# filaPro/unidet3d

Hardware: AMD Instinct MI355X
Metric: scenes/sec fwd+bwd, 100k-pt ScanNet voxel grid, 1/2/4/8 MI355X (higher is better)
Workload: dtype f32

## Files before the change

include/u3d.h:

```cpp
#ifndef U3D_H_
#define U3D_H_

#include <stdint.h>

#ifdef __cplusplus
extern "C" {
#endif

typedef void* u3d_stream_t;

#define U3D_OK 0
#define U3D_EINVAL (-1)
#define U3D_ELAUNCH (-2)
#define U3D_EUNSUPPORTED (-3)

#define U3D_ABI_VERSION 117
int u3d_version(void);
const char* u3d_last_error(void);
int u3d_fp32_math(int mode);

int u3d_conv_kernel(int mode);

int u3d_attn_tile_waves(int waves);

// ... 221 lines not shown
int u3d_attn_varlen_bwd_drop_b16(const void* qkv, const void* out, const void* dout, const float* lse, const int32_t* cu_seqlens,
                                 int B, int max_len, int64_t n_total, int H, int hd, float scale, void* dqkv, float* delta_ws,
                                 double flops_hint, u3d_stream_t stream, double p, uint64_t seed, uint64_t offset);
int u3d_dropout_mask_attn(double p, uint64_t seed, uint64_t offset, int H, int64_t n_total, uint8_t* mask ,
                          u3d_stream_t stream);
int u3d_dropout_mask_rows(double p, uint64_t seed, uint64_t offset, int64_t n, int C, uint8_t* mask , u3d_stream_t stream);
int u3d_dropout_fwd(const float* x, float* y, int64_t n, int C, double p, uint64_t seed, uint64_t offset, u3d_stream_t stream);
int u3d_dropout_bwd(const float* dy, float* dx, int64_t n, int C, double p, uint64_t seed, uint64_t offset, u3d_stream_t stream);
int u3d_dropout_fwd_b16(const void* x, void* y, int64_t n, int C, double p, uint64_t seed, uint64_t offset, u3d_stream_t stream);
int u3d_dropout_bwd_b16(const void* dy, void* dx, int64_t n, int C, double p, uint64_t seed, uint64_t offset, u3d_stream_t stream);

int u3d_gemm_nt(const float* A , const float* W , const float* bias , float* C ,
                int64_t M, int N, int K , const void* w_planes, double flops_hint, u3d_stream_t stream);
#define U3D_BF16_OPERANDS 16
int u3d_linear_act(const float* X , const float* W , const float* bias, int act, float* pre, float* Y ,
                   int64_t M, int N, int K, const void* w_planes, double flops_hint, u3d_stream_t stream);
int u3d_linear_dact(const float* dY , const float* Wt , const float* aux, int act, float* dX ,
                    int64_t M, int N, int K, const void* w_planes, double flops_hint, u3d_stream_t stream);
int u3d_gemm_nt_add(const float* A , const float* W , const float* addend , int flags, float* C, int64_t M,
                    int N, int K, const void* w_planes, double flops_hint, u3d_stream_t stream);
int u3d_ln_linear(const float* X, const float* RES, const float* gamma, const float* beta, float eps, float* SUM, float* NQ, float* STATS,
                  const float* W , const float* bias, int act, float* PRE, float* Y , int64_t M, int C, int N,
                  const void* w_planes, double flops_hint, u3d_stream_t stream);
int u3d_ffn_fwd(const float* X, const float* W1 , const float* b1, const float* W2 , const float* b2,
                int act, float* H, float* A, float* Z , int64_t M, int d_in, int hid, int d_out,
                const void* w1_planes, const void* w2_planes, double flops_hint, u3d_stream_t stream);
int u3d_gelu_fwd(const float* h, float* a, int64_t n, u3d_stream_t stream);
int u3d_gelu_bwd(const float* da, const float* h, float* dh, int64_t n, u3d_stream_t stream);
int u3d_gemm_tn(const float* A , const float* B , float* C , float* colsum_A, int64_t M, int N, int K,
                void* ws, double flops_hint, u3d_stream_t stream);
int u3d_gemm_tn_bf16(const float* A, const float* B, float* C, float* colsum_A, int64_t M, int N, int K, void* ws, double flops_hint,
                     u3d_stream_t stream);
int64_t u3d_gemm_tn_ws_bytes(int64_t M, int N, int K);
int u3d_transpose(const float* in , float* out , int R, int C, u3d_stream_t stream);
int u3d_transpose_batch(const void* desc, int n_desc, int64_t total_blocks, u3d_stream_t stream);
int u3d_weight_planes_batch(const void* desc, int n_desc, int64_t total_blocks, u3d_stream_t stream);

#define U3D_A_BF16 1
#define U3D_B_BF16 2
#define U3D_C_BF16 4
int u3d_gemm_nt_b16(const void* A, const float* W, const float* bias, int epi, const void* aux, void* C, int flags, int64_t M, int N, int K,
                    double flops_hint, u3d_stream_t stream);
int u3d_gemm_tn_b16(const void* A, const void* B, float* C, float* colsum_A, int flags, int64_t M, int N, int K, void* ws, double flops_hint,
                    u3d_stream_t stream);
int64_t u3d_gemm_tn_b16_ws_bytes(int64_t M, int N, int K);
int u3d_gelu_fwd_b16(const void* h, void* a, int64_t n, u3d_stream_t stream);
int u3d_gelu_bwd_b16(const void* da, const void* h, void* dh, int64_t n, u3d_stream_t stream);

#define U3D_GEMM_NATIVE 0
#define U3D_GEMM_X3 1
#define U3D_GEMM_B16 2
int u3d_gemm_nt_plan(int64_t M, int N, int K, int flags, int* kernel, int* tile_m, int* tile_n);
int u3d_gemm_nt_b16_plan(int64_t M, int N, int K, int epi, int flags, int* tile_m, int* tile_n);
int u3d_gemm_tn_plan(int64_t M, int N, int K, int bf16_operands, int* kernel, int* tile_n, int* tile_k, int* splits, int64_t* rows_per_split);
int u3d_gemm_tn_b16_plan(int64_t M, int N, int K, int flags, int* tile_n, int* tile_k, int* splits, int64_t* rows_per_split);

int u3d_layer_norm_fwd(const float* x, const float* res, const float* gamma, const float* beta, int64_t M, int C, float eps,
                       float* sum_out, float* y, float* stats, u3d_stream_t stream);
int u3d_layer_norm_bwd(const float* s, const float* dy, const float* gamma, const float* stats, int64_t M, int C, float* dx,
                       float* dgamma, float* dbeta, void* ws, u3d_stream_t stream);
int u3d_layer_norm_fwd_b16(const float* x, const float* res, const float* gamma, const float* beta, int64_t M, int C, float eps,
                           float* sum_out, float* y, void* y16, float* stats, u3d_stream_t stream);
int u3d_layer_norm_bwd_b16(const float* s, const float* dy, const float* gamma, const float* stats, int64_t M, int C, float* dx, void* dx16,
                           float* dgamma, float* dbeta, void* ws, u3d_stream_t stream);
int u3d_layer_norm_bwd_sum(const float* s, const float* dy, const float* dy2, const float* dy3, const float* gamma, const float* stats,
                           int64_t M, int C, float* dx, void* dx16, float* dgamma, float* dbeta, void* ws, u3d_stream_t stream);
// ... 96 lines not shown
```

unidet3d_amd/_lib.py:

```python
from __future__ import annotations

import ctypes as C
import os

import torch

_HERE = os.path.dirname(os.path.abspath(__file__))
LIB_PATH = os.environ.get('U3D_LIB_PATH') or os.path.join(_HERE, 'csrc', 'libu3d_hip.so')

_vp, _i32, _i64, _f32, _f64 = C.c_void_p, C.c_int, C.c_int64, C.c_float, C.c_double
_u64 = C.c_uint64


class ConvEpilogue(C.Structure):
    _fields_ = [('raw', _vp), ('raw_ld', _i64), ('raw_col', _i64), ('n_act', _i32), ('act', _vp * 2), ('scale', _vp * 2), ('shift', _vp * 2),
                ('act_ld', _i64 * 2), ('act_col', _i64 * 2), ('relu', _i32 * 2)]


PROTOTYPES = {
    'u3d_version': (_i32, []),
    'u3d_last_error': (C.c_char_p, []),
    'u3d_fp32_math': (_i32, [_i32]),
    'u3d_conv_kernel': (_i32, [_i32]),
    'u3d_attn_tile_waves': (_i32, [_i32]),
    'u3d_prof_enable': (_i32, [_i32, _i32]),
    'u3d_prof_collect': (_i32, [_i32, C.POINTER(_f64), C.POINTER(_i64), C.POINTER(_f64)]),
    'u3d_vox_scene_stats': (_i32, [_vp, _vp, _vp, _i32, _i64, _f32, _i32, _vp, _vp, _vp, _vp]),
    'u3d_vox_scene_stats_ws_bytes': (_i64, [_i32]),
    'u3d_index_words': (_i64, [_i32, _i32, _i32, _i32]),
    'u3d_vox_mark': (_i32, [_vp, _vp, _vp, _i32, _i64, _vp, _f32, _i32, _i32, _i32, _i32, _vp, _vp, _vp]),
    'u3d_index_rank': (_i32, [_vp, _i64, _vp, _vp, _vp]),
    'u3d_index_rank_ws_bytes': (_i64, [_i64]),
    'u3d_index_coords': (_i32, [_vp, _vp, _i32, _i32, _i32, _i32, _vp, _vp]),
    'u3d_vox_finalize': (_i32, [_vp, _vp, _i32, _i64, _vp, _vp, _vp, _vp, _i64, _i64, _vp, _vp, _vp, _vp, _i32, _vp, _vp]),
    'u3d_hash_index_slots': (_i64, [_i64]),
    'u3d_hash_index_ws_bytes': (_i64, [_i64]),
    'u3d_hash_index_build': (_i32, [_vp, _i64, _i64, _vp, _vp, _vp, _vp, _i64, _vp, _vp]),
    'u3d_sort_u64': (_i32, [_vp, _i64, _i32, _vp, _vp, _vp, _vp]),
    'u3d_sort_ws_bytes': (_i64, [_i64, _i32]),
    'u3d_hash_index_coords': (_i32, [_vp, _i64, _i32, _i32, _i32, _vp, _vp]),
    'u3d_cells_of_coords': (_i32, [_vp, _i64, _i32, _i32, _i32, _i32, _i32, _vp, _vp]),
    'u3d_vox_finalize_ws_bytes': (_i64, [_i64, _i64]),
    'u3d_subm_rulebook': (_i32, [_vp, _i64, _vp, _vp, _i64, _i32, _i32, _i32, _i32, _vp, _vp, _vp, _vp, _vp]),
    'u3d_subm_rulebook_ws_bytes': (_i64, [_i64]),
    'u3d_index_mark': (_i32, [_vp, _i64, _i32, _i32, _i32, _i32, _vp, _vp]),
    'u3d_down_rulebook': (_i32, [_vp, _i64, _vp, _vp, _i64, _i32, _i32, _i32, _i32, _vp, _vp, _vp, _vp, _vp]),
    'u3d_down_rulebook_ws_bytes': (_i64, [_i64]),
    'u3d_conv_out_shape': (_i32, [C.POINTER(_i32), _i32, _i32, _i32, C.POINTER(_i32)]),
    'u3d_conv_mark': (_i32, [_vp, _i64, C.POINTER(_i32), _i32, _i32, _i32, _i32, _vp, _vp, _vp]),
# ... 68 lines not shown
    'u3d_relu_bwd': (_i32, [_vp, _vp, _i64, _vp, _vp]),
    'u3d_rows_take': (_i32, [_vp, _vp, _i64, _i64, _i32, _vp, _vp]),
    'u3d_rows_take2': (_i32, [_vp, _vp, _i64, _vp, _vp, _i64, _i64, _i32, _vp, _vp]),
    'u3d_segment_gather_sum': (_i32, [_vp, _vp, _vp, _i64, _i32, _i32, _vp, _vp, _vp]),
    'u3d_segment_mean_xyz': (_i32, [_vp, _i32, _vp, _vp, _i64, _vp, _i32, _vp, _i32, _vp, _vp]),
    'u3d_segment_minmax_xyz': (_i32, [_vp, _i32, _vp, _i64, _i32, _vp, _i32, _vp, _i32, _vp, _vp, _vp]),
    'u3d_criterion_packed': (_i32, [_vp] * 11 + [_i32, _i32, _i64, _i32, _i32, _i64, _i64, _i32, _i32, _f32, _f32, _f32, _f32, _f32, _vp, _vp, _vp, _vp, _vp]),
    'u3d_box_decode_fwd': (_i32, [_vp, _vp, _i64, _vp, _vp]),
    'u3d_box_decode_bwd': (_i32, [_vp, _vp, _i64, _vp, _vp]),
    'u3d_box_decode7_fwd': (_i32, [_vp, _vp, _vp, _i64, _vp, _vp]),
    'u3d_box_decode7_bwd': (_i32, [_vp, _vp, _vp, _i64, _vp, _vp]),
    'u3d_criterion_ws_bytes': (_i64, [_i32, _i32, _i64, _i64, _i64]),
    'u3d_criterion_ws_bytes_gt': (_i64, [_i32, _i32, _i64, _i64, _i64, _i32]),
    'u3d_gemm_nt': (_i32, [_vp, _vp, _vp, _vp, _i64, _i32, _i32, _vp, _f64, _vp]),
    'u3d_linear_act': (_i32, [_vp, _vp, _vp, _i32, _vp, _vp, _i64, _i32, _i32, _vp, _f64, _vp]),
    'u3d_linear_dact': (_i32, [_vp, _vp, _vp, _i32, _vp, _i64, _i32, _i32, _vp, _f64, _vp]),
    'u3d_gemm_nt_add': (_i32, [_vp, _vp, _vp, _i32, _vp, _i64, _i32, _i32, _vp, _f64, _vp]),
    'u3d_ln_linear': (_i32, [_vp, _vp, _vp, _vp, _f32, _vp, _vp, _vp, _vp, _vp, _i32, _vp, _vp, _i64, _i32, _i32, _vp, _f64, _vp]),
    'u3d_ffn_fwd': (_i32, [_vp, _vp, _vp, _vp, _vp, _i32, _vp, _vp, _vp, _i64, _i32, _i32, _i32, _vp, _vp, _f64, _vp]),
    'u3d_gelu_fwd': (_i32, [_vp, _vp, _i64, _vp]),
    'u3d_gelu_bwd': (_i32, [_vp, _vp, _vp, _i64, _vp]),
    'u3d_gemm_nt_b16': (_i32, [_vp, _vp, _vp, _i32, _vp, _vp, _i32, _i64, _i32, _i32, _f64, _vp]),
    'u3d_gemm_tn_b16': (_i32, [_vp, _vp, _vp, _vp, _i32, _i64, _i32, _i32, _vp, _f64, _vp]),
    'u3d_gemm_tn_b16_ws_bytes': (_i64, [_i64, _i32, _i32]),
    'u3d_gelu_fwd_b16': (_i32, [_vp, _vp, _i64, _vp]),
    'u3d_gelu_bwd_b16': (_i32, [_vp, _vp, _vp, _i64, _vp]),
    'u3d_gemm_nt_plan': (_i32, [_i64, _i32, _i32, _i32, C.POINTER(_i32), C.POINTER(_i32), C.POINTER(_i32)]),
    'u3d_gemm_nt_b16_plan': (_i32, [_i64, _i32, _i32, _i32, _i32, C.POINTER(_i32), C.POINTER(_i32)]),
    'u3d_gemm_tn_plan': (_i32, [_i64, _i32, _i32, _i32, C.POINTER(_i32), C.POINTER(_i32), C.POINTER(_i32), C.POINTER(_i32), C.POINTER(_i64)]),
    'u3d_gemm_tn_b16_plan': (_i32, [_i64, _i32, _i32, _i32, C.POINTER(_i32), C.POINTER(_i32), C.POINTER(_i32), C.POINTER(_i64)]),
    'u3d_gemm_tn': (_i32, [_vp, _vp, _vp, _vp, _i64, _i32, _i32, _vp, _f64, _vp]),
    'u3d_gemm_tn_bf16': (_i32, [_vp, _vp, _vp, _vp, _i64, _i32, _i32, _vp, _f64, _vp]),
    'u3d_gemm_tn_ws_bytes': (_i64, [_i64, _i32, _i32]),
    'u3d_transpose': (_i32, [_vp, _vp, _i32, _i32, _vp]),
    'u3d_transpose_batch': (_i32, [_vp, _i32, _i64, _vp]),
    'u3d_weight_planes_batch': (_i32, [_vp, _i32, _i64, _vp]),
    'u3d_attn_varlen_fwd': (_i32, [_vp, _vp, _i32, _i32, _i64, _i32, _i32, _f32, _vp, _vp, _f64, _vp]),
    'u3d_attn_varlen_bwd': (_i32, [_vp, _vp, _vp, _vp, _vp, _i32, _i32, _i64, _i32, _i32, _f32, _vp, _vp, _f64, _vp]),
    'u3d_attn_varlen_fwd_bf16': (_i32, [_vp, _vp, _i32, _i32, _i64, _i32, _i32, _f32, _vp, _vp, _f64, _vp]),
    'u3d_attn_varlen_bwd_bf16': (_i32, [_vp, _vp, _vp, _vp, _vp, _i32, _i32, _i64, _i32, _i32, _f32, _vp, _vp, _f64, _vp]),
    'u3d_attn_varlen_fwd_b16': (_i32, [_vp, _vp, _i32, _i32, _i64, _i32, _i32, _f32, _vp, _vp, _f64, _vp]),
    'u3d_attn_varlen_bwd_b16': (_i32, [_vp, _vp, _vp, _vp, _vp, _i32, _i32, _i64, _i32, _i32, _f32, _vp, _vp, _f64, _vp]),
    'u3d_attn_varlen_fwd_drop': (_i32, [_vp, _vp, _i32, _i32, _i64, _i32, _i32, _f32, _vp, _vp, _f64, _vp, _f64, _u64, _u64]),
    'u3d_attn_varlen_bwd_drop': (_i32, [_vp, _vp, _vp, _vp, _vp, _i32, _i32, _i64, _i32, _i32, _f32, _vp, _vp, _f64, _vp, _f64, _u64, _u64]),
    'u3d_attn_varlen_fwd_drop_bf16': (_i32, [_vp, _vp, _i32, _i32, _i64, _i32, _i32, _f32, _vp, _vp, _f64, _vp, _f64, _u64, _u64]),
    'u3d_attn_varlen_bwd_drop_bf16': (_i32, [_vp, _vp, _vp, _vp, _vp, _i32, _i32, _i64, _i32, _i32, _f32, _vp, _vp, _f64, _vp, _f64, _u64, _u64]),
    'u3d_attn_varlen_fwd_drop_b16': (_i32, [_vp, _vp, _i32, _i32, _i64, _i32, _i32, _f32, _vp, _vp, _f64, _vp, _f64, _u64, _u64]),
    'u3d_attn_varlen_bwd_drop_b16': (_i32, [_vp, _vp, _vp, _vp, _vp, _i32, _i32, _i64, _i32, _i32, _f32, _vp, _vp, _f64, _vp, _f64, _u64, _u64]),
    'u3d_dropout_mask_attn': (_i32, [_f64, _u64, _u64, _i32, _i64, _vp, _vp]),
    'u3d_dropout_mask_rows': (_i32, [_f64, _u64, _u64, _i64, _i32, _vp, _vp]),
    'u3d_dropout_fwd': (_i32, [_vp, _vp, _i64, _i32, _f64, _u64, _u64, _vp]),
    'u3d_dropout_bwd': (_i32, [_vp, _vp, _i64, _i32, _f64, _u64, _u64, _vp]),
    'u3d_dropout_fwd_b16': (_i32, [_vp, _vp, _i64, _i32, _f64, _u64, _u64, _vp]),
    'u3d_dropout_bwd_b16': (_i32, [_vp, _vp, _i64, _i32, _f64, _u64, _u64, _vp]),
    'u3d_aug_points': (_i32, [_vp, _i64, _vp, _vp, _vp, _i32, _i64, _vp, C.POINTER(_f32), C.POINTER(_f32), _f32, _vp, _vp, _vp]),
    'u3d_aug_extent_f32': (_i32, [_vp, _vp, _i32, _i64, _vp, _vp]),
    'u3d_aug_extent_f64': (_i32, [_vp, _vp, _i32, _i64, _vp, _vp]),
    'u3d_aug_noise_blur': (_i32, [_vp, _vp, _vp, _i32, _i64, _vp, _vp, _vp]),
    'u3d_aug_noise_blur_ws_bytes': (_i64, [_i64]),
    'u3d_aug_elastic': (_i32, [_vp, _i32, _vp, _i32, _vp, _i32, _i64, _vp, _vp, _vp, _vp, _f64, _f64, _vp]),
    'u3d_relabel_ids': (_i32, [_vp, _i64, _vp, _vp, _vp, _i32, _i64, _vp, _i64, _i32, _vp, _vp, _i32, _vp, _vp, _vp, _vp, _vp, _vp]),
    'u3d_relabel_ids_ws_bytes': (_i64, [_i64]),
    'u3d_aug_remap_ids': (_i32, [_vp, _vp, _i32, _i64, _vp, _vp, _vp]),
    'u3d_aug_sp_masks': (_i32, [_vp, _vp, _vp, _i64, _vp, _i32, _i64, _vp, _vp, _vp, _i64, _i64, _vp, _vp, _vp]),
    'u3d_aug_sp_masks_ws_bytes': (_i64, [_i64, _i64]),
    'u3d_aug_points_dn': (_i32, [_vp, _i64, _vp, _vp, _vp, _i32, _i64, _vp, C.POINTER(_f32), C.POINTER(_f32), C.POINTER(_f32), C.POINTER(_f32),
# ... 80 lines not shown
    if torch.device(device).type != 'cuda':
        return t.to(device)
    return t.pin_memory().to(device, non_blocking=True)


def h2d_pack(specs, device):
    parts, off = [], 0
    for values, dtype in specs:
        t = torch.tensor(values, dtype=dtype).reshape(-1)
        parts.append((t, off))
        off = (off + t.numel() * t.element_size() + 15) // 16 * 16
    host = torch.empty(max(off, 16), dtype=torch.uint8)
    if torch.device(device).type == 'cuda':
        host = host.pin_memory()
    for t, o in parts:
        if t.numel():
            host[o:o + t.numel() * t.element_size()].view(t.dtype).copy_(t)
    dev = host.to(device, non_blocking=True)
    return [dev[o:o + t.numel() * t.element_size()].view(t.dtype) for t, o in parts]


_SCRATCH = {}


def scratch(nbytes: int, device) -> torch.Tensor:
    key = (device, stream())
    t = _SCRATCH.get(key)
    if t is None or t.numel() < nbytes:
        t = torch.empty(max(int(nbytes), 1 << 21), dtype=torch.uint8, device=device)
        _SCRATCH[key] = t
    return t


def prof_enable(cls: int, on: bool):
    call('u3d_prof_enable', cls, 1 if on else 0)


def prof_collect(cls: int):
    ms, n, w = _f64(), _i64(), _f64()
    call('u3d_prof_collect', cls, C.byref(ms), C.byref(n), C.byref(w))
    return ms.value, n.value, w.value
```

unidet3d_amd/csrc/gemm.hip:

```cpp
#include "gemm_common.h"

namespace u3d {

#define U3D_MFMA32(a, b, c) __builtin_amdgcn_mfma_f32_32x32x2f32((a), (b), (c), 0, 0, 0)

constexpr int GLD = GK + 4;


template <int TN, int EPI, int TM = GT>
__global__ __launch_bounds__(256) void gemm_nt_k(const float* __restrict__ A, const float* __restrict__ W, const float* __restrict__ bias,
                                                 float* __restrict__ C, int64_t M, int N, int K, const float* __restrict__ aux,
                                                 float* __restrict__ pre) {
    constexpr int NB = TN / 64, TA = TM / 64;
    __shared__ __attribute__((aligned(16))) float As[2][TM * GLD];
    __shared__ __attribute__((aligned(16))) float Bs[2][TN * GLD];
    const int tid = threadIdx.x, lane = tid & 63;
    const int wave = __builtin_amdgcn_readfirstlane(tid >> 6);
    const int wr = wave >> 1, wc = wave & 1, i32 = lane & 31, kh = lane >> 5;
    const int nt_ = (N + TN - 1) / TN;
    const int64_t wid_ = xcd_swizzle(blockIdx.x, gridDim.x);
    const int64_t m0 = (wid_ / nt_) * TM;
    const int n0 = (int)(wid_ % nt_) * TN;
    const int rows_a = (int)min((int64_t)TM, M - m0), rows_b = min(TN, N - n0);
    const __amdgpu_buffer_rsrc_t rs_a = make_rsrc(A + m0 * K, (int64_t)rows_a * K * 4);
// ... 419 lines not shown
            lstore();
            if (t + 2 < nt) gload(t + 2);
        }
        __syncthreads();
    }
    const int64_t pstride = (int64_t)N * K + (colsum ? N : 0);
    const __amdgpu_buffer_rsrc_t rs_o = make_rsrc(partial + (int64_t)split * pstride, (int64_t)N * K * 4);
#pragma unroll
    for (int b = 0; b < NB; ++b) {
        const int k = k0 + 16 * (wc * NB + b) + t16;
        const int vo = k < K ? ((n0 + 4 * g) * K + k) * 4 : 0x7fffffff;
#pragma unroll
        for (int a = 0; a < NA; ++a)
#pragma unroll
            for (int r = 0; r < 4; ++r) {
                float v = acc[a][b][r] + lo[a][b][r];
                asm volatile("" : "+v"(v));
                __builtin_amdgcn_raw_buffer_store_b32(__builtin_bit_cast(unsigned, v), rs_o, vo, (16 * (wr * NA + a) + r) * K * 4, 0);
            }
    }
    if (colsum && k0 == 0) {
#pragma unroll
        for (int c = 0; c < 4; ++c) csum_s[rowa][ca4 * 4 + c] = cs[c];
        __syncthreads();
        if (tid < TA && n0 + tid < N) {
            float v = 0.f;
#pragma unroll
            for (int r = 0; r < RPA; ++r) v += csum_s[r][tid];
            partial[(int64_t)split * pstride + (int64_t)N * K + n0 + tid] = v;
        }
    }
}


__global__ __launch_bounds__(256) void gemm_tn_bf16_k(const float* __restrict__ A, const float* __restrict__ B, float* __restrict__ partial,
                                                      int colsum, int64_t M, int N, int K, int64_t rows_per_split) {
    __shared__ __attribute__((aligned(16))) __bf16 As[2][TKH * TLH];
    __shared__ __attribute__((aligned(16))) __bf16 Bs[2][TKH * TLH];
    __shared__ float csum_s[8][GT];
    const int tid = threadIdx.x, lane = tid & 63;
    const int wave = __builtin_amdgcn_readfirstlane(tid >> 6);
    const int wr = wave >> 1, wc = wave & 1, i32 = lane & 31, kh = lane >> 5;
    const int n0 = blockIdx.x * GT, k0 = blockIdx.y * GT;
    const int64_t mlo = (int64_t)blockIdx.z * rows_per_split;
    const int64_t mhi = min(M, mlo + rows_per_split);
    const int rows = (int)max((int64_t)0, mhi - mlo);
    const int srow = tid >> 5, sc4 = tid & 31;
    const __amdgpu_buffer_rsrc_t rs_a = make_rsrc(A + mlo * N, (int64_t)rows * N * 4);
    const __amdgpu_buffer_rsrc_t rs_b = make_rsrc(B + mlo * K, (int64_t)rows * K * 4);
    const int va = n0 + sc4 * 4 < N ? (srow * N + n0 + sc4 * 4) * 4 : 0x7fffffff;
    const int vb = k0 + sc4 * 4 < K ? (srow * K + k0 + sc4 * 4) * 4 : 0x7fffffff;
    const bool ca = va != 0x7fffffff, cb = vb != 0x7fffffff;
    f32x4 ra[4], rb[4];
    f32x4 cs = {0.f, 0.f, 0.f, 0.f};
    auto gload = [&](int t) {
#pragma unroll
        for (int j = 0; j < 4; ++j) {
            ra[j] = bload128(rs_a, ca ? va + j * 8 * N * 4 : va, t * (TKH * N * 4));
            rb[j] = bload128(rs_b, cb ? vb + j * 8 * K * 4 : vb, t * (TKH * K * 4));
        }
    };
    auto lstore = [&](int buf) {
#pragma unroll
        for (int j = 0; j < 4; ++j) {
            cs += ra[j];
            *reinterpret_cast<bf16x4*>(&As[buf][(srow + 8 * j) * TLH + sc4 * 4]) = bf16x4{(__bf16)ra[j][0], (__bf16)ra[j][1], (__bf16)ra[j][2], (__bf16)ra[j][3]};
// ... 219 lines not shown
        case 0: launch_nt<0>(A, W, bias, C, M, N, K, aux, pre, plan, s, wplanes); break;
        case 1: launch_nt<1>(A, W, bias, C, M, N, K, aux, pre, plan, s, wplanes); break;
        case 2: launch_nt<2>(A, W, bias, C, M, N, K, aux, pre, plan, s, wplanes); break;
        case 3: launch_nt<3>(A, W, bias, C, M, N, K, aux, pre, plan, s, wplanes); break;
        case 4: launch_nt<4>(A, W, bias, C, M, N, K, aux, pre, plan, s, wplanes); break;
        default: launch_nt<5>(A, W, bias, C, M, N, K, aux, pre, plan, s, wplanes); break;
    }
    return check_launch("gemm_nt");
}

static bool tn_x3_on() { static const int on = [] { const char* e = getenv("U3D_TN_X3"); return e ? atoi(e) : 1; }(); return on != 0 && fp32_x3(); }
static int tn_x3_ta(int N, int K) { return tn_tile(N, K) == GT ? 128 : 64; }
static int tn_x3_splits(int64_t M, int N, int K) {
    const int64_t tiles = ceil_div(N, tn_x3_ta(N, K)) * ceil_div(K, 64);
    return tn_clamp_splits(ceil_div(768, tiles), M, TXK);
}

static int tn_plan(int64_t M, int N, int K, bool bf, TnPlan* plan) {
    if (M <= 0 || N <= 0 || K <= 0) return U3D_EINVAL;
    if (N % 4 || K % 4) { set_error("gemm_tn: N=%d, K=%d must be multiples of 4", N, K); return U3D_EUNSUPPORTED; }
    const bool x3 = !bf && tn_x3_on();
    const int T = bf ? GT : tn_tile(N, K);
    const int S = x3 ? tn_x3_splits(M, N, K) : tn_splits(M, N, K, T, bf);
    const int64_t rps = x3 ? ceil_div(ceil_div(M, S), TXK) * TXK : ceil_div(ceil_div(M, S), GK) * GK;
    if (!tn_offsets_ok("gemm_tn", M, N, K, rps)) return U3D_EUNSUPPORTED;
    plan->kernel = x3 ? U3D_GEMM_X3 : (bf ? U3D_GEMM_B16 : U3D_GEMM_NATIVE);
    plan->ta = x3 ? tn_x3_ta(N, K) : T;
    plan->tb = x3 ? 64 : T;
    plan->splits = S;
    plan->rows_per_split = rps;
    return U3D_OK;
}

}

using namespace u3d;

extern "C" {


int u3d_gemm_nt(const float* A, const float* W, const float* bias, float* C, int64_t M, int N, int K, const void* w_planes, double flops_hint,
                u3d_stream_t stream) {
    return gemm_nt_epi(A, W, bias, C, M, N, K, 0, nullptr, nullptr, w_planes, flops_hint, (hipStream_t)stream);
}

int u3d_linear_act(const float* X, const float* W, const float* bias, int act, float* pre, float* Y, int64_t M, int N, int K,
                   const void* w_planes, double flops_hint, u3d_stream_t stream) {
    const int bf = (act & U3D_BF16_OPERANDS) ? 8 : 0;
    act &= ~U3D_BF16_OPERANDS;
    if (act < 0 || act > 2) return U3D_EINVAL;
    return gemm_nt_epi(X, W, bias, Y, M, N, K, act | bf, nullptr, pre, w_planes, flops_hint, (hipStream_t)stream);
}

int u3d_linear_dact(const float* dY, const float* Wt, const float* aux, int act, float* dX, int64_t M, int N, int K, const void* w_planes,
                    double flops_hint, u3d_stream_t stream) {
    const int bf = (act & U3D_BF16_OPERANDS) ? 8 : 0;
    act &= ~U3D_BF16_OPERANDS;
    if (act < 0 || act > 2) return U3D_EINVAL;
    return gemm_nt_epi(dY, Wt, nullptr, dX, M, N, K, (act == 0 ? 0 : act + 2) | bf, aux, nullptr, w_planes, flops_hint, (hipStream_t)stream);
}

int u3d_gemm_nt_add(const float* A, const float* W, const float* addend, int flags, float* C, int64_t M, int N, int K, const void* w_planes,
                    double flops_hint, u3d_stream_t stream) {
    return gemm_nt_epi(A, W, nullptr, C, M, N, K, 5 | ((flags & U3D_BF16_OPERANDS) ? 8 : 0), addend, nullptr, w_planes, flops_hint, (hipStream_t)stream);
}

// ... 40 lines not shown
        if (plan.ta == 128) hipLaunchKernelGGL((gemm_tn_x3_k<128, 64>), dim3(grid), dim3(256), 0, s, A, B, (float*)ws, colsum_A ? 1 : 0, M, N, K, rps, S);
        else hipLaunchKernelGGL((gemm_tn_x3_k<64, 64>), dim3(grid), dim3(256), 0, s, A, B, (float*)ws, colsum_A ? 1 : 0, M, N, K, rps, S);
    } else if (plan.kernel == U3D_GEMM_B16) hipLaunchKernelGGL(gemm_tn_bf16_k, dim3((unsigned)ceil_div(N, GT), (unsigned)ceil_div(K, GT), S), dim3(256), 0, s, A, B, (float*)ws, colsum_A ? 1 : 0, M, N, K, rps);
    else {
        const unsigned grid = tn_grid(S, N, K, plan.ta, plan.tb);
        if (plan.ta == 64) hipLaunchKernelGGL(gemm_tn_k<64>, dim3(grid), dim3(256), 0, s, A, B, (float*)ws, colsum_A ? 1 : 0, M, N, K, rps, S);
        else hipLaunchKernelGGL(gemm_tn_k<GT>, dim3(grid), dim3(256), 0, s, A, B, (float*)ws, colsum_A ? 1 : 0, M, N, K, rps, S);
    }
    launch_tn_reduce((const float*)ws, S, N, K, C, colsum_A, s);
    return check_launch("gemm_tn");
}

int u3d_gemm_nt_plan(int64_t M, int N, int K, int flags, int* kernel, int* tile_m, int* tile_n) {
    if (flags & ~U3D_BF16_OPERANDS) return U3D_EINVAL;
    NtPlan plan;
    if (const int rc = nt_plan(M, N, K, (flags & U3D_BF16_OPERANDS) != 0, &plan)) return rc;
    if (kernel) *kernel = plan.kernel;
    if (tile_m) *tile_m = NT_TM[plan.tile];
    if (tile_n) *tile_n = NT_TN[plan.tile];
    return U3D_OK;
}

int u3d_gemm_tn_plan(int64_t M, int N, int K, int bf16_operands, int* kernel, int* tile_n, int* tile_k, int* splits, int64_t* rows_per_split) {
    TnPlan plan;
    if (const int rc = tn_plan(M, N, K, bf16_operands != 0, &plan)) return rc;
    if (kernel) *kernel = plan.kernel;
    if (tile_n) *tile_n = plan.ta;
    if (tile_k) *tile_k = plan.tb;
    if (splits) *splits = plan.splits;
    if (rows_per_split) *rows_per_split = plan.rows_per_split;
    return U3D_OK;
}

int u3d_gelu_fwd(const float* h, float* a, int64_t n, u3d_stream_t stream) {
    if (!h || !a || n <= 0 || n % 4) return U3D_EINVAL;
    int64_t g = ceil_div(n / 4, 256);
    hipLaunchKernelGGL(gelu_fwd_k, dim3((unsigned)(g > 8192 ? 8192 : g)), dim3(256), 0, (hipStream_t)stream, (const float4*)h, (float4*)a, n / 4);
    return check_launch("gelu_fwd");
}

int u3d_gelu_bwd(const float* da, const float* h, float* dh, int64_t n, u3d_stream_t stream) {
    if (!da || !h || !dh || n <= 0 || n % 4) return U3D_EINVAL;
    int64_t g = ceil_div(n / 4, 256);
    hipLaunchKernelGGL(gelu_bwd_k, dim3((unsigned)(g > 8192 ? 8192 : g)), dim3(256), 0, (hipStream_t)stream, (const float4*)da, (const float4*)h, (float4*)dh, n / 4);
    return check_launch("gelu_bwd");
}

int u3d_gemm_tn(const float* A, const float* B, float* C, float* colsum_A, int64_t M, int N, int K, void* ws, double flops_hint,
                u3d_stream_t stream) {
    return gemm_tn_impl(A, B, C, colsum_A, M, N, K, ws, flops_hint, stream, false);
}

int u3d_gemm_tn_bf16(const float* A, const float* B, float* C, float* colsum_A, int64_t M, int N, int K, void* ws, double flops_hint,
                     u3d_stream_t stream) {
    return gemm_tn_impl(A, B, C, colsum_A, M, N, K, ws, flops_hint, stream, true);
}

int u3d_transpose(const float* in, float* out, int R, int C, u3d_stream_t stream) {
    if (!in || !out || R <= 0 || C <= 0) return U3D_EINVAL;
    hipLaunchKernelGGL(transpose_k, dim3((C + 31) / 32, (R + 31) / 32), dim3(256), 0, (hipStream_t)stream, in, out, R, C);
    return check_launch("transpose");
}

int u3d_weight_planes_batch(const void* desc, int n_desc, int64_t total_blocks, u3d_stream_t stream) {
    if (!desc || n_desc <= 0 || total_blocks <= 0 || total_blocks >= 0x7fffffffLL) return U3D_EINVAL;
    hipLaunchKernelGGL(planes_batch_k, dim3((unsigned)total_blocks), dim3(256), 0, (hipStream_t)stream, (const PlDesc*)desc, n_desc);
// ... 11 lines not shown
```

unidet3d_amd/dense.py:

```python
from __future__ import annotations

import os

import torch

from . import _lib as L
from . import precision as P
from . import account
from . import wgrad_stream as WS

_PROFILE_FLOPS = False


def set_profile_flops(on: bool):
    global _PROFILE_FLOPS
    _PROFILE_FLOPS = bool(on)


ACT_NONE, ACT_RELU, ACT_GELU = 0, 1, 2
EPI_BIAS, EPI_RELU, EPI_RELU_MASK, EPI_ADD = 0, 1, 3, 5
EPI_GELU_MASK = 4


def _book(M, N, K, nbytes=None, extra_mn=0):
# ... 230 lines not shown
    dx = torch.empty_like(x)
    dg = torch.empty(C, dtype=torch.float32, device=x.device)
    db = torch.empty(C, dtype=torch.float32, device=x.device)
    if M:
        ws = L.scratch(L.lib().u3d_layer_norm_ws_bytes(M, C), x.device)
        L.call('u3d_layer_norm_bwd', L.ptr(x), L.ptr(dy), L.ptr(gamma), L.ptr(stats), M, C, L.ptr(dx), L.ptr(dg), L.ptr(db), L.ptr(ws),
               L.stream())
    else:
        dg.zero_(); db.zero_()
    return dx, dg, db


def _gelu_pass(name, *ts):
    out = torch.empty_like(ts[0])
    if out.numel():
        L.call(name, *[L.ptr(t) for t in ts], L.ptr(out), out.numel(), L.stream())
    return out


def _input_grad(flow, dy, weight, wt=None, wt_planes=None, epi=EPI_BIAS, aux=None, out_bf16=False):
    wt, wt_planes = _transposed(weight, flow.q, wt, wt_planes)
    return flow.nt(_pad_cols(dy, flow.q), wt, None, epi, aux, out_bf16, wt_planes)


def _weight_grad(flow, dy, x, want_bias):
    N = dy.shape[1]
    dyp = _pad_cols(dy, flow.tn_q(dy))
    dw, db = flow.tn(dyp, x, want_bias)
    if dyp is not dy:
        dw, db = dw[:N].contiguous(), (db[:N].contiguous() if db is not None else None)
    return dw, db


def _weight_grad_overlapped(flow, dy, x, want_bias, weight, bias):
    if not (WS.mode() == 2 and _OVERLAP_TN and dy.is_cuda and WS.async_dw_ok(weight, bias)):
        return _weight_grad(flow, dy, x, want_bias)
    _, grads = WS.run_on_side_stream(dy.device, lambda: _weight_grad(flow, dy, x, want_bias), reads=(dy, x))
    WS.queue_join(dy.device)
    return grads


_OVERLAP_TN = os.environ.get('U3D_OVERLAP_TN', '1') != '0'


class _LinearFn(torch.autograd.Function):

    @staticmethod
    def forward(ctx, flow, x, weight, bias, out_bf16):
        x = x.contiguous()
        xa = flow.operand(x)
        w = weight.contiguous()
        ctx.save_for_backward(xa, w)
        ctx.flow = flow
        ctx.has_bias = bias is not None
        ctx.bias_ref = bias
        ctx.wt = _wt_of(weight)
        ctx.wt_planes = _planes_of(ctx.wt)
        ctx.dx_bf16 = x.dtype == torch.bfloat16
        return flow.nt(xa, w, bias, out_bf16=bool(out_bf16) and w.shape[0] % 2 == 0, planes=_planes_of(weight))

    @staticmethod
    def backward(ctx, dy):
        xa, weight = ctx.saved_tensors
        flow = ctx.flow
        dy = dy.contiguous()
        da = flow.operand(dy)
        dx = dw = db = None
# ... 229 lines not shown
```

unidet3d_amd/wgrad_stream.py:

```python
from __future__ import annotations

import os
from typing import Dict

import torch

_MODE = int(os.environ.get('U3D_WGRAD_SIDE_STREAM', '0') or 0)
_N_SIDE = max(1, int(os.environ.get('U3D_SIDE_STREAMS', '1') or 1))
_SIDE: Dict = {}
_SIDE_RR: Dict = {}
_JOIN_PENDING: Dict = {}
_ASYNC_DW_SEEN: Dict = {}


def set_wgrad_overlap(mode: int) -> int:
    global _MODE
    prev, _MODE = _MODE, int(mode)
    return prev


def mode() -> int:
    return _MODE


def _side_stream(device):
    if device not in _SIDE:
        _SIDE[device] = [torch.cuda.Stream(device=device) for _ in range(_N_SIDE)]
        _SIDE_RR[device] = 0
    i = _SIDE_RR[device]
    _SIDE_RR[device] = (i + 1) % len(_SIDE[device])
    return _SIDE[device][i]


def run_on_side_stream(device, launch, reads):
    main = torch.cuda.current_stream(device)
    side = _side_stream(device)
    side.wait_stream(main)
    with torch.cuda.stream(side):
        made = launch()
    for t in reads:
        t.record_stream(side)
    for t in made or ():
        if t is not None:
            t.record_stream(main)
    return side, made


def _pass_id() -> int:
    return torch._C._current_graph_task_id()


def async_dw_ok(*params) -> bool:
    ok = not torch.is_grad_enabled()
    task = _pass_id()
    for w in params:
        if w is None:
            continue
        ok = ok and w.is_leaf and w.grad is None and not getattr(w, '_backward_hooks', None) and \
            not getattr(w, '_post_accumulate_grad_hooks', None) and _ASYNC_DW_SEEN.get(id(w)) != task
    if ok:
        for w in params:
            if w is not None:
                _ASYNC_DW_SEEN[id(w)] = task
    elif any(w is not None and id(w) in _ASYNC_DW_SEEN for w in params):
        join_wgrad_stream()
    return ok


def join_wgrad_stream(device=None):
    for dev in ([device] if device is not None else list(_JOIN_PENDING)):
        if _JOIN_PENDING.pop(dev, None) and dev in _SIDE:
            cur = torch.cuda.current_stream(dev)
            for st in _SIDE[dev]:
                cur.wait_stream(st)


def queue_join(device):
    _JOIN_PENDING[device] = True
    task = _pass_id()
    torch.autograd.Variable._execution_engine.queue_callback(lambda: end_of_backward(device, task))


def end_of_backward(device=None, task=None):
    join_wgrad_stream(device)
    if task is None:
        _ASYNC_DW_SEEN.clear()
    else:
        for k in [k for k, t in _ASYNC_DW_SEEN.items() if t >= task]:
            del _ASYNC_DW_SEEN[k]
```

Baseline: 309.2.

## Batch deferred weight-gradient GEMMs into one grouped split-K launch

Weight-gradient GEMMs for large-row linears are no longer launched one at a time. They are queued during backward and flushed either when a work-unit threshold is reached or before any stream join. The flush runs one grouped three-plane bf16 MFMA kernel plus one reduce kernel, driven by a device-side descriptor table. This targets launch overhead and under-filled grids from many small weight-gradient products, at the cost of extra partial-sum workspace and later materialisation of the gradients.

```diff
diff --git a/include/u3d.h b/include/u3d.h
--- a/include/u3d.h
+++ b/include/u3d.h
@@ -277,6 +277,17 @@
 int u3d_gemm_tn_bf16(const float* A, const float* B, float* C, float* colsum_A, int64_t M, int N, int K, void* ws, double flops_hint,
                      u3d_stream_t stream);
 int64_t u3d_gemm_tn_ws_bytes(int64_t M, int N, int K);
+typedef struct U3dTnDesc {
+    const float* A;
+    const float* B;
+    float* C;
+    float* colsum_A;
+    int64_t M;
+    int32_t N, K;
+} U3dTnDesc;
+int u3d_gemm_tn_group(const U3dTnDesc* desc, int n_desc, void* ws, double flops_hint, u3d_stream_t stream);
+int64_t u3d_gemm_tn_group_ws_bytes(const U3dTnDesc* desc, int n_desc);
+int u3d_gemm_tn_group_plan(int64_t M, int N, int K, int* tile_n, int* tile_k, int* splits, int64_t* rows_per_split);
 int u3d_transpose(const float* in , float* out , int R, int C, u3d_stream_t stream);
 int u3d_transpose_batch(const void* desc, int n_desc, int64_t total_blocks, u3d_stream_t stream);
 int u3d_weight_planes_batch(const void* desc, int n_desc, int64_t total_blocks, u3d_stream_t stream);
diff --git a/unidet3d_amd/_lib.py b/unidet3d_amd/_lib.py
--- a/unidet3d_amd/_lib.py
+++ b/unidet3d_amd/_lib.py
@@ -15,6 +15,10 @@
 class ConvEpilogue(C.Structure):
     _fields_ = [('raw', _vp), ('raw_ld', _i64), ('raw_col', _i64), ('n_act', _i32), ('act', _vp * 2), ('scale', _vp * 2), ('shift', _vp * 2),
                 ('act_ld', _i64 * 2), ('act_col', _i64 * 2), ('relu', _i32 * 2)]
+
+
+class TnDesc(C.Structure):
+    _fields_ = [('A', _vp), ('B', _vp), ('C', _vp), ('colsum_A', _vp), ('M', _i64), ('N', _i32), ('K', _i32)]
 
 
 PROTOTYPES = {
@@ -149,6 +153,9 @@
     'u3d_gemm_tn': (_i32, [_vp, _vp, _vp, _vp, _i64, _i32, _i32, _vp, _f64, _vp]),
     'u3d_gemm_tn_bf16': (_i32, [_vp, _vp, _vp, _vp, _i64, _i32, _i32, _vp, _f64, _vp]),
     'u3d_gemm_tn_ws_bytes': (_i64, [_i64, _i32, _i32]),
+    'u3d_gemm_tn_group': (_i32, [_vp, _i32, _vp, _f64, _vp]),
+    'u3d_gemm_tn_group_ws_bytes': (_i64, [_vp, _i32]),
+    'u3d_gemm_tn_group_plan': (_i32, [_i64, _i32, _i32, C.POINTER(_i32), C.POINTER(_i32), C.POINTER(_i32), C.POINTER(_i64)]),
     'u3d_transpose': (_i32, [_vp, _vp, _i32, _i32, _vp]),
     'u3d_transpose_batch': (_i32, [_vp, _i32, _i64, _vp]),
     'u3d_weight_planes_batch': (_i32, [_vp, _i32, _i64, _vp]),
@@ -295,6 +302,27 @@
     return t
 
 
+TN_GROUP_CALLS = [0, 0]
+
+
+def gemm_tn_group_plan(M: int, N: int, K: int):
+    a, b, s, r = _i32(0), _i32(0), _i32(0), _i64(0)
+    rc = lib().u3d_gemm_tn_group_plan(M, N, K, C.byref(a), C.byref(b), C.byref(s), C.byref(r))
+    return rc, a.value, b.value, s.value, r.value
+
+
+def gemm_tn_group(products, device, flops: float = 0.0):
+    desc = (TnDesc * len(products))()
+    for d, (dy, x, dw, db) in zip(desc, products):
+        d.A, d.B, d.C, d.colsum_A, d.M, d.N, d.K = ptr(dy), ptr(x), ptr(dw), ptr(db), dy.shape[0], dy.shape[1], x.shape[1]
+    nbytes = lib().u3d_gemm_tn_group_ws_bytes(desc, len(products))
+    if nbytes < 0:
+        raise U3DError(f'u3d_gemm_tn_group_ws_bytes failed with code {nbytes}: {lib().u3d_last_error().decode()}')
+    call('u3d_gemm_tn_group', desc, len(products), ptr(scratch(nbytes, device)), flops, stream())
+    TN_GROUP_CALLS[0] += 1
+    TN_GROUP_CALLS[1] += len(products)
+
+
 def prof_enable(cls: int, on: bool):
     call('u3d_prof_enable', cls, 1 if on else 0)
 
diff --git a/unidet3d_amd/csrc/gemm.hip b/unidet3d_amd/csrc/gemm.hip
--- a/unidet3d_amd/csrc/gemm.hip
+++ b/unidet3d_amd/csrc/gemm.hip
@@ -475,6 +475,184 @@
     }
 }
 
+constexpr int TN_GROUP_MAX = 32;
+struct TnGroupProd {
+    const float* A; const float* B; float* partial; float* C; float* colsum;
+    int64_t M;
+    int N, K, ta, splits, rot, unit0, rblock0, rblocks;
+};
+struct TnGroupTable { TnGroupProd p[TN_GROUP_MAX]; int n; };
+
+template <int TA, int TB>
+__device__ __forceinline__ void tn_x3_unit(const float* __restrict__ A, const float* __restrict__ B, float* __restrict__ partial, int colsum,
+                                           int rows, int N, int K, int n0, int k0, __bf16* As, __bf16* Bs, float* csum_s) {
+    constexpr int LA = TA + 16, LB = TB + 16;
+    constexpr int PA = TXK * LA, PB = TXK * LB;
+    constexpr int TPA = TA / 4, TPB = TB / 4;
+    constexpr int RPA = 256 / TPA, RPB = 256 / TPB;
+    constexpr int NPA = TXK / RPA, NPB = TXK / RPB;
+    constexpr int NA = TA / 32, NB = TB / 32;
+    const int tid = threadIdx.x, lane = tid & 63, t16 = lane & 15, g = lane >> 4;
+    const int wave = __builtin_amdgcn_readfirstlane(tid >> 6);
+    const int wr = wave >> 1, wc = wave & 1;
+    const int rowa = tid / TPA, ca4 = tid % TPA, rowb = tid / TPB, cb4 = tid % TPB;
+    const __amdgpu_buffer_rsrc_t rs_a = make_rsrc(A, (int64_t)rows * N * 4);
+    const __amdgpu_buffer_rsrc_t rs_b = make_rsrc(B, (int64_t)rows * K * 4);
+    const int va = n0 + ca4 * 4 < N ? (rowa * N + n0 + ca4 * 4) * 4 : 0x7fffffff;
+    const int vb = k0 + cb4 * 4 < K ? (rowb * K + k0 + cb4 * 4) * 4 : 0x7fffffff;
+    const bool oka = va != 0x7fffffff, okb = vb != 0x7fffffff;
+    f32x4 ra[NPA], rb[NPB];
+    f32x4 cs = {0.f, 0.f, 0.f, 0.f};
+    auto gload = [&](int t) {
+#pragma unroll
+        for (int j = 0; j < NPA; ++j) ra[j] = bload128(rs_a, oka ? va + j * RPA * N * 4 : va, t * (TXK * N * 4));
+#pragma unroll
+        for (int j = 0; j < NPB; ++j) rb[j] = bload128(rs_b, okb ? vb + j * RPB * K * 4 : vb, t * (TXK * K * 4));
+    };
+    auto put = [&](__bf16* tile, int plane, int off, const f32x4& v) {
+        unsigned w0[3], w1[3];
+        split3_pair(v[0], v[1], w0[0], w0[1], w0[2]);
+        split3_pair(v[2], v[3], w1[0], w1[1], w1[2]);
+#pragma unroll
+        for (int q = 0; q < 3; ++q) *reinterpret_cast<uint2*>(tile + q * plane + off) = make_uint2(w0[q], w1[q]);
+    };
+    auto lstore = [&]() {
+#pragma unroll
+        for (int j = 0; j < NPA; ++j) {
+            cs += ra[j];
+            put(As, PA, (rowa + j * RPA) * LA + ca4 * 4, ra[j]);
+        }
+#pragma unroll
+        for (int j = 0; j < NPB; ++j) put(Bs, PB, (rowb + j * RPB) * LB + cb4 * 4, rb[j]);
+    };
+    auto frag = [&](const __bf16* tile, int L, int blk) -> bf16x8 {
+        const __bf16* s0 = tile + (4 * g + (t16 >> 2)) * L + blk * 16 + 4 * (t16 & 3);
+        return tr16_pair(s0, s0 + 16 * L);
+    };
+    f32x4 acc[NA][NB], lo[NA][NB];
+#pragma unroll
+    for (int a = 0; a < NA; ++a)
+#pragma unroll
+        for (int b = 0; b < NB; ++b) { acc[a][b] = f32x4{0.f, 0.f, 0.f, 0.f}; lo[a][b] = acc[a][b]; }
+    const int nt = (rows + TXK - 1) / TXK;
+    if (nt > 0) {
+        gload(0);
+        lstore();
+        if (nt > 1) gload(1);
+    }
+    __syncthreads();
+    for (int t = 0; t < nt; ++t) {
+        bf16x8 fb[NB][3];
+#pragma unroll
+        for (int b = 0; b < NB; ++b)
+#pragma unroll
+            for (int q = 0; q < 3; ++q) fb[b][q] = frag(Bs + q * PB, LB, wc * NB + b);
+#pragma unroll
+        for (int a = 0; a < NA; ++a) {
+            bf16x8 fa[3];
+#pragma unroll
+            for (int q = 0; q < 3; ++q) fa[q] = frag(As + q * PA, LA, wr * NA + a);
+#pragma unroll
+            for (int b = 0; b < NB; ++b) {
+#pragma unroll
+                for (int o = 2; o >= 1; --o)
+#pragma unroll
+                    for (int qa = 0; qa <= o; ++qa)
+                        lo[a][b] = __builtin_amdgcn_mfma_f32_16x16x32_bf16(fa[qa], fb[b][o - qa], lo[a][b], 0, 0, 0);
+                acc[a][b] = __builtin_amdgcn_mfma_f32_16x16x32_bf16(fa[0], fb[b][0], acc[a][b], 0, 0, 0);
+            }
+        }
+        __syncthreads();
+        if (t + 1 < nt) {
+            lstore();
+            if (t + 2 < nt) gload(t + 2);
+        }
+        __syncthreads();
+    }
+    const __amdgpu_buffer_rsrc_t rs_o = make_rsrc(partial, (int64_t)N * K * 4);
+#pragma unroll
+    for (int b = 0; b < NB; ++b) {
+        const int k = k0 + 16 * (wc * NB + b) + t16;
+        const int vo = k < K ? ((n0 + 4 * g) * K + k) * 4 : 0x7fffffff;
+#pragma unroll
+        for (int a = 0; a < NA; ++a)
+#pragma unroll
+            for (int r = 0; r < 4; ++r) {
+                float v = acc[a][b][r] + lo[a][b][r];
+                asm volatile("" : "+v"(v));
+                __builtin_amdgcn_raw_buffer_store_b32(__builtin_bit_cast(unsigned, v), rs_o, vo, (16 * (wr * NA + a) + r) * K * 4, 0);
+            }
+    }
+    if (colsum && k0 == 0) {
+#pragma unroll
+        for (int c = 0; c < 4; ++c) csum_s[rowa * TA + ca4 * 4 + c] = cs[c];
+        __syncthreads();
+        if (tid < TA && n0 + tid < N) {
+            float v = 0.f;
+#pragma unroll
+            for (int r = 0; r < RPA; ++r) v += csum_s[r * TA + tid];
+            partial[(int64_t)N * K + n0 + tid] = v;
+        }
+    }
+}
+
+#define U3D_TN_GROUP_FIND(tab, first, id, lo)                    \
+    int lo = 0;                                                  \
+    for (int hi_ = (tab).n; hi_ - lo > 1;) {                     \
+        const int mid_ = (lo + hi_) >> 1;                        \
+        if ((tab).p[mid_].first <= (int)(id)) lo = mid_; else hi_ = mid_; \
+    }
+
+__global__ __launch_bounds__(256) __attribute__((amdgpu_waves_per_eu(3))) void gemm_tn_x3_group_k(const TnGroupTable tab, int rows_per_split) {
+    __shared__ __attribute__((aligned(16))) __bf16 As[3 * TXK * (128 + 16)];
+    __shared__ __attribute__((aligned(16))) __bf16 Bs[3 * TXK * (64 + 16)];
+    __shared__ float csum_s[8 * 128];
+    U3D_TN_GROUP_FIND(tab, unit0, blockIdx.x, pi)
+    const TnGroupProd& d = tab.p[pi];
+    const int N = d.N, K = d.K, ta = d.ta;
+    const int tiles_n = (N + ta - 1) / ta, tiles = tiles_n * ((K + 63) / 64);
+    const int rem = (int)blockIdx.x - d.unit0;
+    const int slot = rem >> 3, tile = slot % tiles;
+    const int split = (slot / tiles) * 8 + ((rem - d.rot) & 7);
+    if (split >= d.splits) return;
+    const int64_t mlo = (int64_t)split * rows_per_split;
+    const int rows = (int)min((int64_t)rows_per_split, d.M - mlo);
+    const int n0 = (tile % tiles_n) * ta, k0 = (tile / tiles_n) * 64;
+    const int colsum = d.colsum ? 1 : 0;
+    float* part = d.partial + (int64_t)split * ((int64_t)N * K + (colsum ? N : 0));
+    if (ta == 128) tn_x3_unit<128, 64>(d.A + mlo * N, d.B + mlo * K, part, colsum, rows, N, K, n0, k0, As, Bs, csum_s);
+    else tn_x3_unit<64, 64>(d.A + mlo * N, d.B + mlo * K, part, colsum, rows, N, K, n0, k0, As, Bs, csum_s);
+}
+
+__global__ __launch_bounds__(256) void gemm_tn_group_reduce_k(const TnGroupTable tab) {
+    U3D_TN_GROUP_FIND(tab, rblock0, blockIdx.x, pi)
+    const TnGroupProd& d = tab.p[pi];
+    const int S = d.splits;
+    const int64_t n4_main = (int64_t)d.N * d.K / 4, n4 = n4_main + (d.colsum ? d.N / 4 : 0);
+    const float4* partial = reinterpret_cast<const float4*>(d.partial);
+    for (int64_t i = (int64_t)((int)blockIdx.x - d.rblock0) * 256 + threadIdx.x; i < n4; i += (int64_t)d.rblocks * 256) {
+        float4 v[4];
+#pragma unroll
+        for (int u = 0; u < 4; ++u) v[u] = make_float4(0.f, 0.f, 0.f, 0.f);
+        int s = 0;
+        for (; s + 4 <= S; s += 4) {
+#pragma unroll
+            for (int u = 0; u < 4; ++u) {
+                const float4 t = partial[(int64_t)(s + u) * n4 + i];
+                v[u].x += t.x; v[u].y += t.y; v[u].z += t.z; v[u].w += t.w;
+            }
+        }
+        for (; s < S; ++s) {
+            const float4 t = partial[(int64_t)s * n4 + i];
+            v[0].x += t.x; v[0].y += t.y; v[0].z += t.z; v[0].w += t.w;
+        }
+        float4* dst = i < n4_main ? reinterpret_cast<float4*>(d.C) + i : reinterpret_cast<float4*>(d.colsum) + (i - n4_main);
+        *dst = make_float4((v[0].x + v[1].x) + (v[2].x + v[3].x), (v[0].y + v[1].y) + (v[2].y + v[3].y),
+                                                      (v[0].z + v[1].z) + (v[2].z + v[3].z), (v[0].w + v[1].w) + (v[2].w + v[3].w));
+    }
+}
+#undef U3D_TN_GROUP_FIND
+
 
 __global__ __launch_bounds__(256) void gemm_tn_bf16_k(const float* __restrict__ A, const float* __restrict__ B, float* __restrict__ partial,
                                                       int colsum, int64_t M, int N, int K, int64_t rows_per_split) {
@@ -760,6 +938,35 @@
     return U3D_OK;
 }
 
+static int64_t tn_group_rows() {
+    static const int rows = [] {
+        const char* e = getenv("U3D_TN_GROUP_ROWS");
+        const int v = e ? atoi(e) : 0;
+        return v >= TXK && v <= 4096 && v % TXK == 0 ? v : 1024;
+    }();
+    return rows;
+}
+
+static int tn_group_plan(int64_t M, int N, int K, TnPlan* plan) {
+    if (M <= 0 || N <= 0 || K <= 0) return U3D_EINVAL;
+    if (!tn_x3_on()) { set_error("gemm_tn_group: three-plane fp32 math only (u3d_fp32_math = 1, U3D_TN_X3 not 0)"); return U3D_EUNSUPPORTED; }
+    if (N % 4 || K % 4) { set_error("gemm_tn_group: N=%d, K=%d must be multiples of 4", N, K); return U3D_EUNSUPPORTED; }
+    const int64_t rps = tn_group_rows(), S = ceil_div(M, rps);
+    if (!tn_offsets_ok("gemm_tn_group", M, N, K, rps) || S >= (1 << 20)) {
+        if (S >= (1 << 20)) set_error("gemm_tn_group: M=%lld has too many row splits", (long long)M);
+        return U3D_EUNSUPPORTED;
+    }
+    plan->kernel = U3D_GEMM_X3;
+    plan->ta = tn_x3_ta(N, K);
+    plan->tb = 64;
+    plan->splits = (int)S;
+    plan->rows_per_split = rps;
+    return U3D_OK;
+}
+static int64_t tn_group_partial_bytes(const TnPlan& plan, int N, int K, bool colsum) {
+    return ceil_div((int64_t)plan.splits * ((int64_t)N * K + (colsum ? N : 0)) * 4, 256) * 256;
+}
+
 }
 
 using namespace u3d;
@@ -866,6 +1073,67 @@
     return U3D_OK;
 }
 
+int u3d_gemm_tn_group_plan(int64_t M, int N, int K, int* tile_n, int* tile_k, int* splits, int64_t* rows_per_split) {
+    TnPlan plan;
+    if (const int rc = tn_group_plan(M, N, K, &plan)) return rc;
+    if (tile_n) *tile_n = plan.ta;
+    if (tile_k) *tile_k = plan.tb;
+    if (splits) *splits = plan.splits;
+    if (rows_per_split) *rows_per_split = plan.rows_per_split;
+    return U3D_OK;
+}
+
+static int tn_group_check(const U3dTnDesc* desc, int n_desc, int64_t* bytes) {
+    if (!desc || n_desc <= 0) return U3D_EINVAL;
+    int64_t total = 0, units = 0;
+    for (int i = 0; i < n_desc; ++i) {
+        const U3dTnDesc& d = desc[i];
+        if (!d.A || !d.B || !d.C) return U3D_EINVAL;
+        TnPlan plan;
+        if (const int rc = tn_group_plan(d.M, d.N, d.K, &plan)) return rc;
+        total += tn_group_partial_bytes(plan, d.N, d.K, d.colsum_A != nullptr);
+        units += ceil_div((int64_t)plan.splits, 8) * 8 * ceil_div(d.N, plan.ta) * ceil_div(d.K, plan.tb);
+        if (units >= 0x7fffffffLL) { set_error("gemm_tn_group: too many work units in one table"); return U3D_EUNSUPPORTED; }
+    }
+    if (bytes) *bytes = total;
+    return U3D_OK;
+}
+
+int64_t u3d_gemm_tn_group_ws_bytes(const U3dTnDesc* desc, int n_desc) {
+    int64_t bytes = 0;
+    const int rc = tn_group_check(desc, n_desc, &bytes);
+    return rc ? rc : bytes + 256;
+}
+
+int u3d_gemm_tn_group(const U3dTnDesc* desc, int n_desc, void* ws, double flops_hint, u3d_stream_t stream) {
+    if (!ws) return U3D_EINVAL;
+    if (const int rc = tn_group_check(desc, n_desc, nullptr)) return rc;
+    hipStream_t s = (hipStream_t)stream;
+    ProfScope prof(U3D_K_GEMM, s, flops_hint);
+    char* part = (char*)ws;
+    int rot = 0;
+    for (int first = 0; first < n_desc; first += TN_GROUP_MAX) {
+        TnGroupTable tab;
+        tab.n = n_desc - first < TN_GROUP_MAX ? n_desc - first : TN_GROUP_MAX;
+        int64_t units = 0, rblocks = 0;
+        for (int i = 0; i < tab.n; ++i) {
+            const U3dTnDesc& d = desc[first + i];
+            TnPlan plan;
+            tn_group_plan(d.M, d.N, d.K, &plan);
+            const int64_t n4 = ((int64_t)d.N * d.K + (d.colsum_A ? d.N : 0)) / 4;
+            const int64_t rb = ceil_div(n4, 256) > 1024 ? 1024 : ceil_div(n4, 256);
+            tab.p[i] = TnGroupProd{d.A, d.B, (float*)part, d.C, d.colsum_A, d.M, d.N, d.K, plan.ta, plan.splits, rot, (int)units, (int)rblocks, (int)rb};
+            units += tn_grid(plan.splits, d.N, d.K, plan.ta, plan.tb);
+            rblocks += rb;
+            rot = (rot + plan.splits) & 7;
+            part += tn_group_partial_bytes(plan, d.N, d.K, d.colsum_A != nullptr);
+        }
+        hipLaunchKernelGGL(gemm_tn_x3_group_k, dim3((unsigned)units), dim3(256), 0, s, tab, (int)tn_group_rows());
+        hipLaunchKernelGGL(gemm_tn_group_reduce_k, dim3((unsigned)rblocks), dim3(256), 0, s, tab);
+    }
+    return check_launch("gemm_tn_group");
+}
+
 int u3d_gelu_fwd(const float* h, float* a, int64_t n, u3d_stream_t stream) {
     if (!h || !a || n <= 0 || n % 4) return U3D_EINVAL;
     int64_t g = ceil_div(n / 4, 256);
diff --git a/unidet3d_amd/dense.py b/unidet3d_amd/dense.py
--- a/unidet3d_amd/dense.py
+++ b/unidet3d_amd/dense.py
@@ -286,7 +286,70 @@
     return dw, db
 
 
+_TN_GROUP = os.environ.get('U3D_TN_GROUP', '1') != '0'
+_TN_GROUP_MIN_ROWS = 4096
+_TN_GROUP_FLUSH_UNITS = int(os.environ.get('U3D_TN_GROUP_FLUSH', '768') or 0)
+
+
+class _TnQueue:
+    items = []
+    units = 0
+    flops = 0.0
+    task = None
+    device = None
+
+
+def _tn_group_units(flow, dy, x):
+    M, N = dy.shape
+    K = x.shape[1]
+    if not (_TN_GROUP and flow is FP32 and dy.is_cuda and M >= _TN_GROUP_MIN_ROWS and N >= 64 and K >= 64 and N % 4 == 0 and K % 4 == 0):
+        return 0
+    rc, ta, tk, splits, _ = L.gemm_tn_group_plan(M, N, K)
+    return 0 if rc else splits * (-(-N // ta)) * (-(-K // tk))
+
+
+def flush_weight_grads():
+    q = _TnQueue
+    if not q.items:
+        return
+    items, flops, dev = q.items, q.flops, q.device
+    q.items, q.units, q.flops, q.task = [], 0, 0.0, None
+    if WS.mode() == 2 and _OVERLAP_TN:
+        reads = [t for it in items for t in it if t is not None]
+        WS.run_on_side_stream(dev, lambda: L.gemm_tn_group(items, dev, flops), reads=reads)
+        WS.side_launched(dev)
+    else:
+        L.gemm_tn_group(items, dev, flops)
+
+
+WS.on_join(flush_weight_grads)
+
+
+def _queue_weight_grad(dy, x, want_bias, units):
+    q = _TnQueue
+    task = WS._pass_id()
+    if q.items and (q.task != task or q.device != dy.device):
+        flush_weight_grads()
+    M, N = dy.shape
+    K = x.shape[1]
+    dw = torch.empty(N, K, dtype=torch.float32, device=dy.device)
+    db = torch.empty(N, dtype=torch.float32, device=dy.device) if want_bias else None
+    q.items.append((dy, x, dw.detach(), db.detach() if db is not None else None))
+    q.units += units
+    q.flops += _book(M, N, K)
+    q.task, q.device = task, dy.device
+    WS.queue_join(dy.device, launched=False)
+    if _TN_GROUP_FLUSH_UNITS and q.units >= _TN_GROUP_FLUSH_UNITS:
+        flush_weight_grads()
+    return dw, db
+
+
 def _weight_grad_overlapped(flow, dy, x, want_bias, weight, bias):
+    units = _tn_group_units(flow, dy, x)
+    if units:
+        if WS._pass_id() != -1 and WS.async_dw_ok(weight, bias):
+            return _queue_weight_grad(dy, x, want_bias, units)
+        return _weight_grad(flow, dy, x, want_bias)
     if not (WS.mode() == 2 and _OVERLAP_TN and dy.is_cuda and WS.async_dw_ok(weight, bias)):
         return _weight_grad(flow, dy, x, want_bias)
     _, grads = WS.run_on_side_stream(dy.device, lambda: _weight_grad(flow, dy, x, want_bias), reads=(dy, x))
diff --git a/unidet3d_amd/wgrad_stream.py b/unidet3d_amd/wgrad_stream.py
--- a/unidet3d_amd/wgrad_stream.py
+++ b/unidet3d_amd/wgrad_stream.py
@@ -11,6 +11,7 @@
 _SIDE_RR: Dict = {}
 _JOIN_PENDING: Dict = {}
 _ASYNC_DW_SEEN: Dict = {}
+_BEFORE_JOIN = []
 
 
 def set_wgrad_overlap(mode: int) -> int:
@@ -33,6 +34,8 @@
 
 
 def run_on_side_stream(device, launch, reads):
+    for flush in _BEFORE_JOIN:
+        flush()
     main = torch.cuda.current_stream(device)
     side = _side_stream(device)
     side.wait_stream(main)
@@ -68,6 +71,8 @@
 
 
 def join_wgrad_stream(device=None):
+    for flush in _BEFORE_JOIN:
+        flush()
     for dev in ([device] if device is not None else list(_JOIN_PENDING)):
         if _JOIN_PENDING.pop(dev, None) and dev in _SIDE:
             cur = torch.cuda.current_stream(dev)
@@ -75,8 +80,17 @@
                 cur.wait_stream(st)
 
 
-def queue_join(device):
+def on_join(flush):
+    _BEFORE_JOIN.append(flush)
+
+
+def side_launched(device):
     _JOIN_PENDING[device] = True
+
+
+def queue_join(device, launched=True):
+    if launched:
+        _JOIN_PENDING[device] = True
     task = _pass_id()
     torch.autograd.Variable._execution_engine.queue_callback(lambda: end_of_backward(device, task))
 
```

Result: slower. 263.3 (-14.9%).
